# adajel/KNP-EMI-DG

Hardware: AMD Instinct MI355X
Metric: DoF-updates/sec per PDE timestep (higher is better)
Workload: dtype f64; 1 GPU; 3D idealized 4-axon mesh r=2 (995328 tets, 11943936 P1-DG DoFs: phi + K,Cl solved, Na eliminated), HH membranes + stimulus, full splitting step; parallelism=slab1

## Files before the change

### knp-emi-dg_amd/csrc/apply_ring.hip

```cpp
#include "cell_geom.hpp"
#include "ring_common.hpp"
#include "ring_facet.hpp"
#include <algorithm>
#include <cstdlib>
#include <map>

namespace {

using namespace ring;
constexpr int RH = 224;
constexpr int RHX = RH / 32;
constexpr int RENT = RB + RH;
constexpr int RSLOTS = 3;
constexpr int RLISTB = 1024;
constexpr int RNLIST = 4;
constexpr int RLOADERS = 4;
constexpr int META_F = 0, META_L = 1024, META_N = 3072, META_C = 4096, META_M = 5120, META_KNP = 6144, META_EMI = 5120;
constexpr int RCLS = 43;

__device__ __forceinline__ void dma_list(const MeshDev& m, int64_t b, unsigned dst, int lane) {
    const int off = lane * 4 < m.hb_stride ? lane * 4 : 0;
    glds16(m.hb_src + b * m.hb_stride + off, dst);
}
template <int NTHREADS> __device__ __forceinline__ void stage_class_records(const MeshDev& m, double* s_cls) {
    for (int i = threadIdx.x; i < m.ncls * 11; i += NTHREADS) s_cls[(i / 11) * RCLS + (i % 11)] = m.cls_table[(i / 11) * KNP_CLS_STRIDE + (i % 11)];
    for (int i = threadIdx.x; i < m.ncls * KNP_CLS_EXT; i += NTHREADS) s_cls[(i / KNP_CLS_EXT) * RCLS + 11 + (i % KNP_CLS_EXT)] = m.cls_ext[i];
}

template <int NS> struct KnpRing {
    static constexpr int XB = RENT * 32;
    static constexpr int G0 = NS * XB;
    static constexpr int GH0 = G0 + RB * 32;
    static constexpr int META0 = GH0 + 4096;
    static constexpr int SLOT = META0 + META_KNP;
    static constexpr int NDATA = NS * 8 + NS * RHX + 8 + 4 + 6;
    static_assert(NDATA <= 63, "vmcnt is a 6-bit counter");
};

struct CellMeta { uint32_t flags, nm; uint2 lw; unsigned cls, mymat; };
__device__ __forceinline__ CellMeta read_meta(const char* meta, unsigned t, bool knp) {
    CellMeta q;
    q.flags = ((const lds_u32*)(meta + META_F))[t];
    q.lw.x = ((const lds_u32*)(meta + META_L))[2 * t];
    q.lw.y = ((const lds_u32*)(meta + META_L))[2 * t + 1];
    q.cls = ((const lds_u16*)(meta + META_C))[t];
    q.nm = 0; q.mymat = 0;
    if (knp) {
        q.nm = ((const lds_u32*)(meta + META_N))[t];
        q.mymat = ((const lds_u8*)(meta + META_M))[t];
    }
    return q;
}

template <int NS, int NG>
__global__ __launch_bounds__(RB * NG + 64 * RLOADERS) void k_knp_apply_ring(MeshDev m, const double* __restrict__ x, const double* __restrict__ gphi,
                                                                 double* __restrict__ yout, KnpArgs ka, const uint8_t* __restrict__ mat,
                                                                 const uint8_t* __restrict__ nmat4, const double* __restrict__ dtab, int dbg) {
    typedef KnpRing<NS> R;
    constexpr int NV = 4, KS = NS / NG, NTHREADS = RB * NG + 64 * RLOADERS;
    static_assert(KS * NG == NS, "species split evenly over the consumer groups");
    extern __shared__ __attribute__((aligned(16))) char smem[];
    char* s_list = smem + RSLOTS * R::SLOT;
    double* s_cls = reinterpret_cast<double*>(s_list + RNLIST * RLISTB);
    double* s_D = s_cls + m.ncls * RCLS;
    const unsigned base = __builtin_amdgcn_readfirstlane((unsigned)(size_t)(lds_char*)smem);
    const unsigned list0 = base + RSLOTS * R::SLOT;
    const int wave = __builtin_amdgcn_readfirstlane((int)(threadIdx.x >> 6));
    const int lane = threadIdx.x & 63;
    const RingWalk w(m);
    if (w.blk(0) < 0) return;
    stage_class_records<NTHREADS>(m, s_cls);
    if (threadIdx.x < NS * KNP_MAX_MAT) s_D[threadIdx.x] = dtab[threadIdx.x];
    if (wave >= 4 * NG) {
        const int lw = wave - 4 * NG;
        constexpr int N0 = 8 + 3, N1 = (NS > 1 ? 8 : 0) + 3, N2 = 8 + 4, N3 = NS * RHX;
        auto list_dma = [&](int64_t n) {
            const int64_t b = w.blk(n);
            if (lw == 0 && b >= 0) dma_list(m, b, list0 + (unsigned)(n & (RNLIST - 1)) * RLISTB, lane);
        };
        auto data_dma = [&](int64_t n) {
            const int64_t b = w.blk(n);
            if (dbg & 4) return;
            const unsigned slot = base + (unsigned)(n % RSLOTS) * R::SLOT;
            const lds_int* L = (const lds_int*)(s_list + (n & (RNLIST - 1)) * RLISTB);
            const int64_t c0 = b * RB;
            if (lw == 0) {
                dma_own_rows(x, c0, m.nc, slot, lane);
                glds16(m.fflag + c0 + 4 * lane, slot + R::META0 + META_F);
                glds16(m.hb_loc + (c0 + 2 * lane) * 4, slot + R::META0 + META_L);
                glds16(m.hb_loc + (c0 + 128 + 2 * lane) * 4, slot + R::META0 + META_L + 1024);
            } else if (lw == 1) {
                if (NS > 1) dma_own_rows(x + m.nc * NV, c0, m.nc, slot + R::XB, lane);
                glds16(m.cls + c0 + 8 * lane, slot + R::META0 + META_C);
                glds16(nmat4 + (c0 + 4 * lane) * 4, slot + R::META0 + META_N);
                glds16(mat + c0 + 16 * lane, slot + R::META0 + META_M);
            } else if (lw == 2) {
                dma_own_rows(gphi, c0, m.nc, slot + R::G0, lane);
#pragma unroll
                for (int p = 0; p < 4; ++p) {
                    const int e = p * 64 + lane;
                    const int src = e < m.hb_stride ? L[e] : -1;
                    int64_t Kp = src >= 0 ? (int64_t)(src >> 2) : 0;
                    const int j = src >= 0 ? (src & 3) : 0;
                    if (dbg & 1) Kp = c0 + e < m.nc ? c0 + e : 0;
                    glds16(gphi + Kp * NV + (j >> 1) * 2, slot + R::GH0 + p * 1024);
                }
            } else {
#pragma unroll
                for (int p = 0; p < RHX; ++p) {
                    int64_t Kp = list_cell(L, p * 32 + (lane >> 1), m.hb_stride);
                    if (dbg & 1) Kp = c0 + p * 32 + (lane >> 1) < m.nc ? c0 + p * 32 + (lane >> 1) : 0;
#pragma unroll
                    for (int k = 0; k < NS; ++k) glds16(x + (int64_t)k * m.nc * NV + Kp * NV + swz_half(lane), slot + k * R::XB + RB * 32 + p * 1024);
                }
            }
        };
        load_two_ahead_counted<false, N0, N1, N2, N3>(w, lw, list_dma, data_dma);
        return;
    }
    const unsigned t = threadIdx.x & (RB - 1);
    const int k0 = (wave >> 2) * KS;
    double zpsi[KS];
#pragma unroll
    for (int k = 0; k < KS; ++k) zpsi[k] = ka.z[k0 + k] * ka.psi;
    ring_barrier();
    ring_barrier();
    for (int64_t n = 0;; ++n) {
        const int64_t b = w.blk(n);
        if (b < 0) break;
        const int64_t c = b * RB + t;
        if (c >= m.c_begin && c < m.c_end) {
            const char* slot = smem + (n % RSLOTS) * R::SLOT;
            const CellMeta cur = read_meta(slot + R::META0, t, true);
            const lds_double* X = (const lds_double*)slot + k0 * (RENT * NV);
            const lds_double* G = (const lds_double*)(slot + R::G0);
            const lds_double* rec = TO_LDS(s_cls) + cur.cls * RCLS;
            const lds_double* sD = TO_LDS(s_D) + k0 * KNP_MAX_MAT;
            CellGeom<3> K;
            class_gram<3>(rec, K);
            double xv[KS][NV], y[KS][NV], gp[NV], Dk[KS];
            lds_row(G, t, gp);
#pragma unroll
            for (int k = 0; k < KS; ++k) {
                lds_row(X + k * (RENT * NV), t, xv[k]);
                Dk[k] = sD[k * KNP_MAX_MAT + cur.mymat];
            }
            double gx[KS][NV], hvD[KS];
            knp_cell_term<KS>(K, xv, gp, Dk, zpsi, ka.inv_dt, gx, hvD, y);
            const ClassCoef ft{rec + 11};
            if (!(dbg & 2)) {
            knp_facet_ring<KS, 0, RENT * NV>(K, cur.flags, cur.lw.x & 0xffffu, ft, cur.nm & 0xffu, xv, gx, gp, Dk, hvD, zpsi, ka.tau, X, G, sD, y);
            knp_facet_ring<KS, 1, RENT * NV>(K, cur.flags, cur.lw.x >> 16, ft, (cur.nm >> 8) & 0xffu, xv, gx, gp, Dk, hvD, zpsi, ka.tau, X, G, sD, y);
            knp_facet_ring<KS, 2, RENT * NV>(K, cur.flags, cur.lw.y & 0xffffu, ft, (cur.nm >> 16) & 0xffu, xv, gx, gp, Dk, hvD, zpsi, ka.tau, X, G, sD, y);
            knp_facet_ring<KS, 3, RENT * NV>(K, cur.flags, cur.lw.y >> 16, ft, cur.nm >> 24, xv, gx, gp, Dk, hvD, zpsi, ka.tau, X, G, sD, y);
            }
#pragma unroll
            for (int k = 0; k < KS; ++k) store_nodal<3>(yout + (int64_t)(k0 + k) * m.nc * NV, c, y[k]);
        }
        ring_barrier();
    }
}

struct EmiRing {
    static constexpr int XB = RENT * 32;
    static constexpr int META0 = 2 * XB;
    static constexpr int SLOT = META0 + META_EMI;
    static constexpr int NDATA = 8 + 8 + 2 * RHX + 4;
};

constexpr int EMI_SLOTS = 4;
__global__ __launch_bounds__(2 * RB + 64 * RLOADERS) void k_emi_apply_ring(MeshDev m, const double* __restrict__ x, const double* __restrict__ kappa,
                                                                double* __restrict__ yout, double C_phi, double tau) {
    typedef EmiRing R;
    constexpr int NV = 4, NTHREADS = 2 * RB + 64 * RLOADERS;
    extern __shared__ __attribute__((aligned(16))) char smem[];
    char* s_list = smem + EMI_SLOTS * R::SLOT;
    double* s_cls = reinterpret_cast<double*>(s_list + RNLIST * RLISTB);
    const unsigned base = __builtin_amdgcn_readfirstlane((unsigned)(size_t)(lds_char*)smem);
    const unsigned list0 = base + EMI_SLOTS * R::SLOT;
    const int wave = __builtin_amdgcn_readfirstlane((int)(threadIdx.x >> 6));
    const int lane = threadIdx.x & 63;
    const RingWalk w(m);
    if (w.blk(0) < 0) return;
    stage_class_records<NTHREADS>(m, s_cls);
    if (wave >= 8) {
        const int lw = wave - 8;
        constexpr int N0 = 8, N1 = 8, N2 = RHX + 2, N3 = RHX + 2;
        auto list_dma = [&](int64_t n) {
            const int64_t b = w.blk(n);
            if (lw == 0 && b >= 0) dma_list(m, b, list0 + (unsigned)(n & (RNLIST - 1)) * RLISTB, lane);
        };
        auto data_dma = [&](int64_t n) {
            const int64_t c0 = w.blk(n) * RB;
            const unsigned slot = base + (unsigned)(n & (EMI_SLOTS - 1)) * R::SLOT;
            const lds_int* L = (const lds_int*)(s_list + (n & (RNLIST - 1)) * RLISTB);
            if (lw == 0) dma_own_rows(x, c0, m.nc, slot, lane);
            else if (lw == 1) dma_own_rows(kappa, c0, m.nc, slot + R::XB, lane);
            else {
                const double* v = lw == 2 ? x : kappa;
                const unsigned dst = slot + (lw == 2 ? 0 : R::XB) + RB * 32;
#pragma unroll
                for (int p = 0; p < RHX; ++p) glds16(v + list_cell(L, p * 32 + (lane >> 1), m.hb_stride) * NV + swz_half(lane), dst + p * 1024);
                if (lw == 2) {
                    glds16(m.fflag + c0 + 4 * lane, slot + R::META0 + META_F);
                    glds16(m.cls + c0 + 8 * lane, slot + R::META0 + META_C);
                } else {
                    glds16(m.hb_loc + (c0 + 2 * lane) * 4, slot + R::META0 + META_L);
                    glds16(m.hb_loc + (c0 + 128 + 2 * lane) * 4, slot + R::META0 + META_L + 1024);
                }
            }
        };
        load_two_ahead_counted<true, N0, N1, N2, N3>(w, lw, list_dma, data_dma);
        return;
    }
    const unsigned t = threadIdx.x & (RB - 1);
    const int g = wave >> 2;
    ring_barrier();
    ring_barrier();
    CellGeom<3> K;
    double xv[NV], kv[NV], yv[NV], gx[NV];
    const lds_double *X = nullptr, *KA = nullptr;
    ClassCoef ft{nullptr};
    CellMeta cur;
    cur.flags = 0; cur.lw = make_uint2(0u, 0u); cur.cls = 0; cur.nm = 0; cur.mymat = 0;
    int64_t ccur = -1;
    bool valid = false;
    for (int64_t n = 0;; ++n) {
        const int64_t b = w.blk(n);
        if ((n & 1) == g) {
            if (b >= 0) {
                ccur = b * RB + t;
                valid = ccur >= m.c_begin && ccur < m.c_end;
                if (valid) {
                    const char* slot = smem + (n & (EMI_SLOTS - 1)) * R::SLOT;
                    cur = read_meta(slot + R::META0, t, false);
                    X = (const lds_double*)slot;
                    KA = (const lds_double*)(slot + R::XB);
                    const lds_double* rec = TO_LDS(s_cls) + cur.cls * RCLS;
                    ft.ft = rec + 11;
                    class_gram<3>(rec, K);
                    lds_row(X, t, xv);
                    lds_row(KA, t, kv);
                    emi_cell_term(K, xv, kv, gx, yv);
                    emi_facet_ring<0>(K, cur.flags, cur.lw.x & 0xffffu, ft, xv, gx, kv, C_phi, tau, X, KA, yv);
                    emi_facet_ring<1>(K, cur.flags, cur.lw.x >> 16, ft, xv, gx, kv, C_phi, tau, X, KA, yv);
                }
            }
        } else if (n >= 1 && valid) {
            emi_facet_ring<2>(K, cur.flags, cur.lw.y & 0xffffu, ft, xv, gx, kv, C_phi, tau, X, KA, yv);
            emi_facet_ring<3>(K, cur.flags, cur.lw.y >> 16, ft, xv, gx, kv, C_phi, tau, X, KA, yv);
            store_nodal<3>(yout, ccur, yv);
        }
        ring_barrier();
        if (b < 0) break;
    }
}

}

static size_t ring_lds_bytes(const knp_ctx* c, int which) {
    const size_t tables = RNLIST * RLISTB + sizeof(double) * (size_t)c->m.ncls * RCLS;
    if (which == 0) return (size_t)EMI_SLOTS * EmiRing::SLOT + tables;
    const size_t slot = c->p.n_sys == 1 ? KnpRing<1>::SLOT : KnpRing<2>::SLOT;
    return (size_t)RSLOTS * slot + tables + sizeof(double) * (size_t)c->p.n_sys * KNP_MAX_MAT;
}

bool ring_usable(const knp_ctx* c, int which) {
    if (c->degree != 1 || c->m.dim != 3 || !c->m.cls || c->m.ncls > CLS_MAX_LDS || !c->m.hb_src || c->m.hb_stride <= 0 || c->m.hb_stride > RH) return false;
    if (env_int("KNP_APPLY_RING", 1) == 0 || ring_lds_bytes(c, which) > RING_MAX_LDS) return false;
    if (which == 0) return env_int("KNP_EMI_RING", 1) != 0;
    return c->nmat > 0 && c->p.n_sys <= 2 && env_int("KNP_APPLY_MAT", 1) != 0 && env_int("KNP_APPLY_HALO", 1) != 0;
}

int ring_emi_apply(knp_ctx* c, const MeshDev& m, const double* x, const double* kappa, double* y, int reserve_cus) {
    const size_t lds = ring_lds_bytes(c, 0);
    if (!grant_lds(c, k_emi_apply_ring, lds)) { c->err = "hipFuncSetAttribute(k_emi_apply_ring) failed"; return -2; }
    hipLaunchKernelGGL(k_emi_apply_ring, ring_grid(c, m, reserve_cus), dim3(2 * RB + 64 * RLOADERS), lds, c->stream, m, x, kappa, y, c->p.C_phi, c->p.tau_emi);
    HIPCHK(c, hipGetLastError());
    return 0;
}

int ring_knp_apply(knp_ctx* c, const MeshDev& m, const double* x, const double* gphi, double* y, const KnpArgs& ka, int reserve_cus) {
    const int ns = c->p.n_sys;
    const size_t lds = ring_lds_bytes(c, 1);
    const dim3 g = ring_grid(c, m, reserve_cus);
    const bool split = ns == 2 && env_int("KNP_RING_SPLIT", 0) != 0;
#define RING_KNP_LAUNCH(NS_, NG_)                                                                                                     \
    do {                                                                                                                              \
        if (!grant_lds(c, k_knp_apply_ring<NS_, NG_>, lds)) { c->err = "hipFuncSetAttribute(k_knp_apply_ring) failed"; return -2; }  \
        hipLaunchKernelGGL((k_knp_apply_ring<NS_, NG_>), g, dim3(RB * NG_ + 64 * RLOADERS), lds, c->stream, m, x, gphi, y, ka, (const uint8_t*)c->mat,  \
                           (const uint8_t*)c->nmat4, (const double*)c->dtab, env_int("KNP_RING_DEBUG", 0));                     \
    } while (0)
    if (ns == 1) RING_KNP_LAUNCH(1, 1);
    else if (split) RING_KNP_LAUNCH(2, 2);
    else RING_KNP_LAUNCH(2, 1);
#undef RING_KNP_LAUNCH
    HIPCHK(c, hipGetLastError());
    return 0;
}
```

### knp-emi-dg_amd/csrc/ring_facet.hpp

```cpp
#pragma once
#include "ring_common.hpp"

namespace ring {


struct ClassCoef {
    const lds_double* ft;
    template <int I> __device__ __forceinline__ double area(const CellGeom<3>&) const { return ft[8 * I + 6]; }
    template <int I> __device__ __forceinline__ void coef(const CellGeom<3>&, double& gr, double* cf, double& pen_geo, double& nLI_DV) const {
        gr = ft[8 * I];
        pen_geo = ft[8 * I + 4];
        nLI_DV = ft[8 * I + 5];
#pragma unroll
        for (int mm = 0; mm < 3; ++mm) cf[mm] = ft[8 * I + 1 + mm];
    }
};

__device__ __forceinline__ void lds_vertex(const lds_double* co, unsigned v, double* X) {
    typedef double __attribute__((ext_vector_type(2))) vdouble2;
    typedef __attribute__((address_space(3))) vdouble2 lds_vdouble2;
    const vdouble2 a = *(const lds_vdouble2*)(co + 4 * v);
    X[0] = a.x; X[1] = a.y; X[2] = co[4 * v + 2];
}
struct CoordCoef {
    const lds_double* co;
    unsigned vapex;
    double hinv;
    template <int I> __device__ __forceinline__ double area(const CellGeom<3>& K) const { return fast_sqrt(K.G[I][I]) * (3.0 * K.vol); }
    template <int I> __device__ __forceinline__ void coef(const CellGeom<3>& K, double& gr, double* cf, double& pen_geo, double& nLI_DV) const {
        double Xo[3], L[4];
        lds_vertex(co, vapex, Xo);
        apex_bary<3>(K, Xo, L);
        gr = K.G[I][I] * fast_rcp(L[I]);
#pragma unroll
        for (int mm = 0; mm < 3; ++mm) cf[mm] = fma(-L[mm + (mm >= I)], gr, K.G[mm + (mm >= I)][I]);
        const double DV = 3.0 * K.vol;
        pen_geo = hinv * area<I>(K);
        nLI_DV = -L[I] * DV;
    }
};

__device__ __forceinline__ void emi_cell_term(const CellGeom<3>& K, const double* xv, const double* kv, double* gx, double* y) {
    constexpr int NV = 4;
    double kbar = 0.0;
#pragma unroll
    for (int a = 0; a < NV; ++a) kbar += kv[a];
    kbar *= K.vol / (double)NV;
#pragma unroll
    for (int a = 0; a < NV; ++a) {
        double sa = 0.0;
#pragma unroll
        for (int bb = 0; bb < NV; ++bb) sa = fma(xv[bb], K.G[bb][a], sa);
        gx[a] = sa;
        y[a] = kbar * sa;
    }
}

template <int I, typename Coef>
__device__ __forceinline__ void emi_facet_ring(const CellGeom<3>& K, uint32_t flags, unsigned loc, const Coef& src, const double* xv, const double* gx,
                                               const double* kv, double C_phi, double tau, const lds_double* X, const lds_double* KA, double* y) {
    constexpr int D = 3, NV = 4;
    const uint32_t fb = (flags >> (8 * I)) & 0xffu;
    const uint32_t kind = (fb >> 2) & 3u;
    if (kind >= FK_EXTERIOR) return;
    const unsigned j = fb & 3u;
    double xr[NV], kr[NV], xf[D], knf[D];
    lds_row(X, loc, xr);
    lds_row(KA, loc, kr);
    const double xap = pick_apex<D>(xr, (int)j);
#pragma unroll
    for (int mm = 0; mm < D; ++mm) {
        xf[mm] = pick_facet<D>(xr, mm, (int)j);
        knf[mm] = pick_facet<D>(kr, mm, (int)j);
    }
    double du[D], sdu = 0.0;
#pragma unroll
    for (int mm = 0; mm < D; ++mm) {
        du[mm] = xv[mm + (mm >= I)] - xf[mm];
        sdu += du[mm];
    }
    if (kind == FK_MEMBRANE) {
        const double w = C_phi * src.template area<I>(K) * FacetConst<D>::mass;
#pragma unroll
        for (int mm = 0; mm < D; ++mm) y[mm + (mm >= I)] = fma(w, sdu + du[mm], y[mm + (mm >= I)]);
        return;
    }
    double gr, cf[D], pen_geo, nLI_DV;
    src.template coef<I>(K, gr, cf, pen_geo, nLI_DV);
    const double s_own = gx[I];
    double s_nb = xap * gr;
#pragma unroll
    for (int mm = 0; mm < D; ++mm) s_nb = fma(xf[mm], cf[mm], s_nb);
    double kf[D], sk = 0.0, skn = 0.0, q = 0.0;
#pragma unroll
    for (int mm = 0; mm < D; ++mm) {
        kf[mm] = kv[mm + (mm >= I)];
        sk += kf[mm];
        skn += knf[mm];
        q = fma(kf[mm], sdu + du[mm], q);
    }
    const double hm = 0.5 * (double)D * K.vol * FacetConst<D>::mass;
    q *= hm;
#pragma unroll
    for (int a = 0; a < NV; ++a) y[a] = fma(K.G[a][I], q, y[a]);
    const double pw = tau * pen_geo * FacetConst<D>::trip;
    double kb[D], skb = 0.0, skd = 0.0;
#pragma unroll
    for (int mm = 0; mm < D; ++mm) {
        kb[mm] = 0.5 * (kf[mm] + knf[mm]);
        skb += kb[mm];
        skd = fma(kb[mm], du[mm], skd);
    }
    const double bs = fma(skb, sdu, skd);
#pragma unroll
    for (int mm = 0; mm < D; ++mm) {
        const double t1 = hm * fma(s_own, sk + kf[mm], s_nb * (skn + knf[mm]));
        const double t3 = pw * (bs + fma(kb[mm], sdu, du[mm] * fma(2.0, kb[mm], skb)));
        y[mm + (mm >= I)] += t1 + t3;
    }
}

template <int NS>
__device__ __forceinline__ void knp_cell_term(const CellGeom<3>& K, const double (*xv)[4], const double* gp, const double* Dk, const double* zpsi,
                                              double inv_dt, double (*gx)[4], double* hvD, double (*y)[4]) {
    constexpr int NV = 4;
    const double mw = inv_dt * K.vol / 20.0;
#pragma unroll
    for (int k = 0; k < NS; ++k) hvD[k] = 0.5 * K.vol * Dk[k];
#pragma unroll
    for (int k = 0; k < NS; ++k) {
        double sx = 0.0;
#pragma unroll
        for (int a = 0; a < NV; ++a) sx += xv[k][a];
        const double drift = zpsi[k] * Dk[k] * K.vol * sx / (double)NV;
        const double dv = Dk[k] * K.vol;
#pragma unroll
        for (int a = 0; a < NV; ++a) {
            double sacc = 0.0;
#pragma unroll
            for (int bb = 0; bb < NV; ++bb) sacc = fma(xv[k][bb], K.G[bb][a], sacc);
            gx[k][a] = sacc;
            y[k][a] = fma(mw, sx + xv[k][a], fma(dv, sacc, drift * gp[a]));
        }
    }
}

template <int NS, int I, int XS, typename Coef>
__device__ __forceinline__ void knp_facet_ring(const CellGeom<3>& K, uint32_t flags, unsigned loc, const Coef& src, unsigned dsel, const double (*xv)[4],
                                               const double (*gx)[4], const double* gp, const double* Dk, const double* hvD, const double* zpsi,
                                               double tau, const lds_double* X, const lds_double* G, const lds_double* sD, double (*y)[4]) {
    constexpr int D = 3, NV = 4;
    const uint32_t fb = (flags >> (8 * I)) & 0xffu;
    if (((fb >> 2) & 3u) != FK_SIPG) return;
    const unsigned j = fb & 3u;
    double gr, cf[D], pen_geo, nLI_DV;
    src.template coef<I>(K, gr, cf, pen_geo, nLI_DV);
    double gp_nb;
    {
        typedef double __attribute__((ext_vector_type(2))) vdouble2;
        typedef __attribute__((address_space(3))) vdouble2 lds_vdouble2;
        const unsigned idx = loc < (unsigned)RB ? loc * NV + 2u * (((j >> 1) ^ (loc >> 3)) & 1u) : (unsigned)(RB * NV) + (loc - RB) * 2u;
        const vdouble2 g2 = *(const lds_vdouble2*)(G + idx);
        gp_nb = (j & 1u) ? g2.y : g2.x;
    }
    const double DV = (double)D * K.vol;
    const double up_own = fmax(-gp[I], 0.0) * DV;
    const double up_nb = fmax(-gp_nb, 0.0) * nLI_DV;
    const double penA = tau * pen_geo;
    const double hv = 0.5 * K.vol;
#pragma unroll
    for (int k = 0; k < NS; ++k) {
        double xr[NV], xf[D];
        lds_row(X + (unsigned)k * XS, loc, xr);
        const double xap = pick_apex<D>(xr, (int)j);
#pragma unroll
        for (int mm = 0; mm < D; ++mm) xf[mm] = pick_facet<D>(xr, mm, (int)j);
        const double Dn = sD[(unsigned)k * KNP_MAX_MAT + dsel];
        const double s_own = gx[k][I];
        double s_nb = xap * gr;
#pragma unroll
        for (int mm = 0; mm < D; ++mm) s_nb = fma(xf[mm], cf[mm], s_nb);
        const double zp = zpsi[k];
        const double c_own = Dk[k] * fma(-zp, up_own, penA);
        const double c_nb = Dn * fma(-zp, up_nb, penA);
        double sdu = 0.0, w[D], sw = 0.0;
#pragma unroll
        for (int mm = 0; mm < D; ++mm) {
            const double xo = xv[k][mm + (mm >= I)];
            sdu += xo - xf[mm];
            w[mm] = fma(c_own, xo, -c_nb * xf[mm]);
            sw += w[mm];
        }
        const double t1m = fma(FacetConst<D>::mass, sw, hv * fma(Dk[k], s_own, Dn * s_nb));
        const double t2 = hvD[k] * sdu;
#pragma unroll
        for (int a = 0; a < NV; ++a) y[k][a] = fma(K.G[a][I], t2, y[k][a]);
#pragma unroll
        for (int mm = 0; mm < D; ++mm) y[k][mm + (mm >= I)] += fma(FacetConst<D>::mass, w[mm], t1m);
    }
}

}
```

Measured before the change: 2.255 billion DoF/s.

## Software-pipeline LDS neighbor loads ahead of facet compute in ring apply kernels

Splits the KNP and EMI facet routines into a load phase (neighbor rows, diffusion coefficients, class coefficients read from LDS into registers) and a compute phase, then issues each facet's loads one facet ahead of the previous facet's arithmetic. Loads are now issued unconditionally, using the cell's own row when the facet is inactive. The loader waves also read all list entries up front before issuing the global-to-LDS copies, and hoist the swizzle offset. The aim is to hide LDS latency behind the FMA work, at the cost of more registers and possibly lower occupancy.

New measurement: 2.251 billion DoF/s. About the same (-0.2%).

```diff
diff --git a/knp-emi-dg_amd/csrc/apply_ring.hip b/knp-emi-dg_amd/csrc/apply_ring.hip
--- a/knp-emi-dg_amd/csrc/apply_ring.hip
+++ b/knp-emi-dg_amd/csrc/apply_ring.hip
@@ -21,6 +21,17 @@
 __device__ __forceinline__ void dma_list(const MeshDev& m, int64_t b, unsigned dst, int lane) {
     const int off = lane * 4 < m.hb_stride ? lane * 4 : 0;
     glds16(m.hb_src + b * m.hb_stride + off, dst);
+}
+template <int N, int STEP> __device__ __forceinline__ void list_entries(const lds_int* L, int e0, int hs, int* src) {
+    static_assert((N - 1) * STEP + 64 <= RLISTB / 4, "list reads stay inside the list buffer");
+#pragma unroll
+    for (int p = 0; p < N; ++p) src[p] = L[e0 + p * STEP];
+#pragma unroll
+    for (int p = 0; p < N; ++p) src[p] = e0 + p * STEP < hs ? src[p] : -1;
+}
+template <int N, int STEP> __device__ __forceinline__ void own_entries(int64_t c0, int e0, int64_t nc, int* src) {
+#pragma unroll
+    for (int p = 0; p < N; ++p) src[p] = c0 + e0 + p * STEP < nc ? (int)(c0 + e0 + p * STEP) << 2 : 0;
 }
 template <int NTHREADS> __device__ __forceinline__ void stage_class_records(const MeshDev& m, double* s_cls) {
     for (int i = threadIdx.x; i < m.ncls * 11; i += NTHREADS) s_cls[(i / 11) * RCLS + (i % 11)] = m.cls_table[(i / 11) * KNP_CLS_STRIDE + (i % 11)];
@@ -50,6 +61,21 @@
         q.mymat = ((const lds_u8*)(meta + META_M))[t];
     }
     return q;
+}
+
+__device__ __forceinline__ unsigned meta_loc(const CellMeta& q, int I) { return ((I < 2 ? q.lw.x : q.lw.y) >> (16 * (I & 1))) & 0xffffu; }
+template <int KS, int I>
+__device__ __forceinline__ void knp_facet_load(const CellMeta& q, unsigned t, const lds_double* ft, const lds_double* X, const lds_double* G,
+                                               const lds_double* sD, KnpFacetRows<KS>& r, ClassCoef& fc) {
+    const bool on = facet_kind(q.flags, I) == FK_SIPG;
+    fc.load<I>(ft);
+    knp_facet_rows<KS, RENT * 4>(on ? meta_loc(q, I) : t, (q.flags >> (8 * I)) & 3u, on ? (q.nm >> (8 * I)) & 0xffu : q.mymat, X, G, sD, r);
+}
+template <int I>
+__device__ __forceinline__ void emi_facet_load(const CellMeta& q, unsigned t, const lds_double* ft, const lds_double* X, const lds_double* KA,
+                                               EmiFacetRows& r, ClassCoef& fc) {
+    fc.load<I>(ft);
+    emi_facet_rows(facet_kind(q.flags, I) < FK_EXTERIOR ? meta_loc(q, I) : t, X, KA, r);
 }
 
 template <int NS, int NG>
@@ -78,6 +104,7 @@
             const int64_t b = w.blk(n);
             if (lw == 0 && b >= 0) dma_list(m, b, list0 + (unsigned)(n & (RNLIST - 1)) * RLISTB, lane);
         };
+        const double* xrow = x + swz_half(lane);
         auto data_dma = [&](int64_t n) {
             const int64_t b = w.blk(n);
             if (dbg & 4) return;
@@ -96,22 +123,24 @@
                 glds16(mat + c0 + 16 * lane, slot + R::META0 + META_M);
             } else if (lw == 2) {
                 dma_own_rows(gphi, c0, m.nc, slot + R::G0, lane);
+                int src[4];
+                list_entries<4, 64>(L, lane, m.hb_stride, src);
+                if (dbg & 1) own_entries<4, 64>(c0, lane, m.nc, src);
 #pragma unroll
                 for (int p = 0; p < 4; ++p) {
-                    const int e = p * 64 + lane;
-                    const int src = e < m.hb_stride ? L[e] : -1;
-                    int64_t Kp = src >= 0 ? (int64_t)(src >> 2) : 0;
-                    const int j = src >= 0 ? (src & 3) : 0;
-                    if (dbg & 1) Kp = c0 + e < m.nc ? c0 + e : 0;
+                    const int64_t Kp = src[p] >= 0 ? (int64_t)(src[p] >> 2) : 0;
+                    const int j = src[p] >= 0 ? (src[p] & 3) : 0;
                     glds16(gphi + Kp * NV + (j >> 1) * 2, slot + R::GH0 + p * 1024);
                 }
             } else {
+                int src[RHX];
+                list_entries<RHX, 32>(L, lane >> 1, m.hb_stride, src);
+                if (dbg & 1) own_entries<RHX, 32>(c0, lane >> 1, m.nc, src);
 #pragma unroll
                 for (int p = 0; p < RHX; ++p) {
-                    int64_t Kp = list_cell(L, p * 32 + (lane >> 1), m.hb_stride);
-                    if (dbg & 1) Kp = c0 + p * 32 + (lane >> 1) < m.nc ? c0 + p * 32 + (lane >> 1) : 0;
-#pragma unroll
-                    for (int k = 0; k < NS; ++k) glds16(x + (int64_t)k * m.nc * NV + Kp * NV + swz_half(lane), slot + k * R::XB + RB * 32 + p * 1024);
+                    const int64_t Kp = src[p] >= 0 ? (int64_t)(src[p] >> 2) : 0;
+#pragma unroll
+                    for (int k = 0; k < NS; ++k) glds16(xrow + (int64_t)k * m.nc * NV + Kp * NV, slot + k * R::XB + RB * 32 + p * 1024);
                 }
             }
         };
@@ -145,14 +174,20 @@
                 lds_row(X + k * (RENT * NV), t, xv[k]);
                 Dk[k] = sD[k * KNP_MAX_MAT + cur.mymat];
             }
+            KnpFacetRows<KS> nb[4];
+            ClassCoef fc[4];
+            const bool facets = !(dbg & 2);
+            if (facets) knp_facet_load<KS, 0>(cur, t, rec + 11, X, G, sD, nb[0], fc[0]);
             double gx[KS][NV], hvD[KS];
             knp_cell_term<KS>(K, xv, gp, Dk, zpsi, ka.inv_dt, gx, hvD, y);
-            const ClassCoef ft{rec + 11};
-            if (!(dbg & 2)) {
-            knp_facet_ring<KS, 0, RENT * NV>(K, cur.flags, cur.lw.x & 0xffffu, ft, cur.nm & 0xffu, xv, gx, gp, Dk, hvD, zpsi, ka.tau, X, G, sD, y);
-            knp_facet_ring<KS, 1, RENT * NV>(K, cur.flags, cur.lw.x >> 16, ft, (cur.nm >> 8) & 0xffu, xv, gx, gp, Dk, hvD, zpsi, ka.tau, X, G, sD, y);
-            knp_facet_ring<KS, 2, RENT * NV>(K, cur.flags, cur.lw.y & 0xffffu, ft, (cur.nm >> 16) & 0xffu, xv, gx, gp, Dk, hvD, zpsi, ka.tau, X, G, sD, y);
-            knp_facet_ring<KS, 3, RENT * NV>(K, cur.flags, cur.lw.y >> 16, ft, cur.nm >> 24, xv, gx, gp, Dk, hvD, zpsi, ka.tau, X, G, sD, y);
+            if (facets) {
+                knp_facet_load<KS, 1>(cur, t, rec + 11, X, G, sD, nb[1], fc[1]);
+                if (facet_kind(cur.flags, 0) == FK_SIPG) knp_facet_terms<KS, 0>(K, cur.flags, fc[0], nb[0], xv, gx, gp, Dk, hvD, zpsi, ka.tau, y);
+                knp_facet_load<KS, 2>(cur, t, rec + 11, X, G, sD, nb[2], fc[2]);
+                if (facet_kind(cur.flags, 1) == FK_SIPG) knp_facet_terms<KS, 1>(K, cur.flags, fc[1], nb[1], xv, gx, gp, Dk, hvD, zpsi, ka.tau, y);
+                knp_facet_load<KS, 3>(cur, t, rec + 11, X, G, sD, nb[3], fc[3]);
+                if (facet_kind(cur.flags, 2) == FK_SIPG) knp_facet_terms<KS, 2>(K, cur.flags, fc[2], nb[2], xv, gx, gp, Dk, hvD, zpsi, ka.tau, y);
+                if (facet_kind(cur.flags, 3) == FK_SIPG) knp_facet_terms<KS, 3>(K, cur.flags, fc[3], nb[3], xv, gx, gp, Dk, hvD, zpsi, ka.tau, y);
             }
 #pragma unroll
             for (int k = 0; k < KS; ++k) store_nodal<3>(yout + (int64_t)(k0 + k) * m.nc * NV, c, y[k]);
@@ -197,10 +232,12 @@
             if (lw == 0) dma_own_rows(x, c0, m.nc, slot, lane);
             else if (lw == 1) dma_own_rows(kappa, c0, m.nc, slot + R::XB, lane);
             else {
-                const double* v = lw == 2 ? x : kappa;
+                const double* v = (lw == 2 ? x : kappa) + swz_half(lane);
                 const unsigned dst = slot + (lw == 2 ? 0 : R::XB) + RB * 32;
-#pragma unroll
-                for (int p = 0; p < RHX; ++p) glds16(v + list_cell(L, p * 32 + (lane >> 1), m.hb_stride) * NV + swz_half(lane), dst + p * 1024);
+                int src[RHX];
+                list_entries<RHX, 32>(L, lane >> 1, m.hb_stride, src);
+#pragma unroll
+                for (int p = 0; p < RHX; ++p) glds16(v + (src[p] >= 0 ? (int64_t)(src[p] >> 2) : 0) * NV, dst + p * 1024);
                 if (lw == 2) {
                     glds16(m.fflag + c0 + 4 * lane, slot + R::META0 + META_F);
                     glds16(m.cls + c0 + 8 * lane, slot + R::META0 + META_C);
@@ -219,8 +256,9 @@
     ring_barrier();
     CellGeom<3> K;
     double xv[NV], kv[NV], yv[NV], gx[NV];
-    const lds_double *X = nullptr, *KA = nullptr;
-    ClassCoef ft{nullptr};
+    EmiFacetRows nb[4];
+    ClassCoef fc[4];
+    const lds_double *X3 = nullptr, *rec3 = nullptr;
     CellMeta cur;
     cur.flags = 0; cur.lw = make_uint2(0u, 0u); cur.cls = 0; cur.nm = 0; cur.mymat = 0;
     int64_t ccur = -1;
@@ -234,21 +272,25 @@
                 if (valid) {
                     const char* slot = smem + (n & (EMI_SLOTS - 1)) * R::SLOT;
                     cur = read_meta(slot + R::META0, t, false);
-                    X = (const lds_double*)slot;
-                    KA = (const lds_double*)(slot + R::XB);
+                    const lds_double* X = (const lds_double*)slot;
+                    const lds_double* KA = (const lds_double*)(slot + R::XB);
                     const lds_double* rec = TO_LDS(s_cls) + cur.cls * RCLS;
-                    ft.ft = rec + 11;
+                    X3 = X; rec3 = rec + 11;
                     class_gram<3>(rec, K);
                     lds_row(X, t, xv);
                     lds_row(KA, t, kv);
+                    emi_facet_load<0>(cur, t, rec + 11, X, KA, nb[0], fc[0]);
                     emi_cell_term(K, xv, kv, gx, yv);
-                    emi_facet_ring<0>(K, cur.flags, cur.lw.x & 0xffffu, ft, xv, gx, kv, C_phi, tau, X, KA, yv);
-                    emi_facet_ring<1>(K, cur.flags, cur.lw.x >> 16, ft, xv, gx, kv, C_phi, tau, X, KA, yv);
+                    emi_facet_load<1>(cur, t, rec + 11, X, KA, nb[1], fc[1]);
+                    if (facet_kind(cur.flags, 0) < FK_EXTERIOR) emi_facet_terms<0>(K, cur.flags, fc[0], nb[0], xv, gx, kv, C_phi, tau, yv);
+                    emi_facet_load<2>(cur, t, rec + 11, X, KA, nb[2], fc[2]);
+                    if (facet_kind(cur.flags, 1) < FK_EXTERIOR) emi_facet_terms<1>(K, cur.flags, fc[1], nb[1], xv, gx, kv, C_phi, tau, yv);
                 }
             }
         } else if (n >= 1 && valid) {
-            emi_facet_ring<2>(K, cur.flags, cur.lw.y & 0xffffu, ft, xv, gx, kv, C_phi, tau, X, KA, yv);
-            emi_facet_ring<3>(K, cur.flags, cur.lw.y >> 16, ft, xv, gx, kv, C_phi, tau, X, KA, yv);
+            emi_facet_load<3>(cur, t, rec3, X3, X3 + R::XB / 8, nb[3], fc[3]);
+            if (facet_kind(cur.flags, 2) < FK_EXTERIOR) emi_facet_terms<2>(K, cur.flags, fc[2], nb[2], xv, gx, kv, C_phi, tau, yv);
+            if (facet_kind(cur.flags, 3) < FK_EXTERIOR) emi_facet_terms<3>(K, cur.flags, fc[3], nb[3], xv, gx, kv, C_phi, tau, yv);
             store_nodal<3>(yout, ccur, yv);
         }
         ring_barrier();
diff --git a/knp-emi-dg_amd/csrc/ring_facet.hpp b/knp-emi-dg_amd/csrc/ring_facet.hpp
--- a/knp-emi-dg_amd/csrc/ring_facet.hpp
+++ b/knp-emi-dg_amd/csrc/ring_facet.hpp
@@ -5,16 +5,21 @@
 
 
 struct ClassCoef {
-    const lds_double* ft;
-    template <int I> __device__ __forceinline__ double area(const CellGeom<3>&) const { return ft[8 * I + 6]; }
+    double v[7];
+    template <int I> __device__ __forceinline__ void load(const lds_double* ft) {
+#pragma unroll
+        for (int i = 0; i < 7; ++i) v[i] = ft[8 * I + i];
+    }
+    template <int I> __device__ __forceinline__ double area(const CellGeom<3>&) const { return v[6]; }
     template <int I> __device__ __forceinline__ void coef(const CellGeom<3>&, double& gr, double* cf, double& pen_geo, double& nLI_DV) const {
-        gr = ft[8 * I];
-        pen_geo = ft[8 * I + 4];
-        nLI_DV = ft[8 * I + 5];
-#pragma unroll
-        for (int mm = 0; mm < 3; ++mm) cf[mm] = ft[8 * I + 1 + mm];
+        gr = v[0];
+        pen_geo = v[4];
+        nLI_DV = v[5];
+#pragma unroll
+        for (int mm = 0; mm < 3; ++mm) cf[mm] = v[1 + mm];
     }
 };
+__device__ __forceinline__ uint32_t facet_kind(uint32_t flags, int I) { return (flags >> (8 * I + 2)) & 3u; }
 
 __device__ __forceinline__ void lds_vertex(const lds_double* co, unsigned v, double* X) {
     typedef double __attribute__((ext_vector_type(2))) vdouble2;
@@ -56,17 +61,20 @@
     }
 }
 
+struct EmiFacetRows { double xr[4], kr[4]; };
+__device__ __forceinline__ void emi_facet_rows(unsigned loc, const lds_double* X, const lds_double* KA, EmiFacetRows& r) {
+    lds_row(X, loc, r.xr);
+    lds_row(KA, loc, r.kr);
+}
 template <int I, typename Coef>
-__device__ __forceinline__ void emi_facet_ring(const CellGeom<3>& K, uint32_t flags, unsigned loc, const Coef& src, const double* xv, const double* gx,
-                                               const double* kv, double C_phi, double tau, const lds_double* X, const lds_double* KA, double* y) {
+__device__ __forceinline__ void emi_facet_terms(const CellGeom<3>& K, uint32_t flags, const Coef& src, const EmiFacetRows& r, const double* xv,
+                                                const double* gx, const double* kv, double C_phi, double tau, double* y) {
     constexpr int D = 3, NV = 4;
     const uint32_t fb = (flags >> (8 * I)) & 0xffu;
     const uint32_t kind = (fb >> 2) & 3u;
-    if (kind >= FK_EXTERIOR) return;
     const unsigned j = fb & 3u;
-    double xr[NV], kr[NV], xf[D], knf[D];
-    lds_row(X, loc, xr);
-    lds_row(KA, loc, kr);
+    const double *xr = r.xr, *kr = r.kr;
+    double xf[D], knf[D];
     const double xap = pick_apex<D>(xr, (int)j);
 #pragma unroll
     for (int mm = 0; mm < D; ++mm) {
@@ -118,6 +126,14 @@
         const double t3 = pw * (bs + fma(kb[mm], sdu, du[mm] * fma(2.0, kb[mm], skb)));
         y[mm + (mm >= I)] += t1 + t3;
     }
+}
+template <int I, typename Coef>
+__device__ __forceinline__ void emi_facet_ring(const CellGeom<3>& K, uint32_t flags, unsigned loc, const Coef& src, const double* xv, const double* gx,
+                                               const double* kv, double C_phi, double tau, const lds_double* X, const lds_double* KA, double* y) {
+    if (facet_kind(flags, I) >= FK_EXTERIOR) return;
+    EmiFacetRows r;
+    emi_facet_rows(loc, X, KA, r);
+    emi_facet_terms<I>(K, flags, src, r, xv, gx, kv, C_phi, tau, y);
 }
 
 template <int NS>
@@ -145,24 +161,33 @@
     }
 }
 
-template <int NS, int I, int XS, typename Coef>
-__device__ __forceinline__ void knp_facet_ring(const CellGeom<3>& K, uint32_t flags, unsigned loc, const Coef& src, unsigned dsel, const double (*xv)[4],
-                                               const double (*gx)[4], const double* gp, const double* Dk, const double* hvD, const double* zpsi,
-                                               double tau, const lds_double* X, const lds_double* G, const lds_double* sD, double (*y)[4]) {
-    constexpr int D = 3, NV = 4;
-    const uint32_t fb = (flags >> (8 * I)) & 0xffu;
-    if (((fb >> 2) & 3u) != FK_SIPG) return;
-    const unsigned j = fb & 3u;
-    double gr, cf[D], pen_geo, nLI_DV;
-    src.template coef<I>(K, gr, cf, pen_geo, nLI_DV);
-    double gp_nb;
+template <int NS> struct KnpFacetRows { double xr[NS][4], g2[2], Dn[NS]; };
+template <int NS, int XS>
+__device__ __forceinline__ void knp_facet_rows(unsigned loc, unsigned j, unsigned dsel, const lds_double* X, const lds_double* G, const lds_double* sD,
+                                               KnpFacetRows<NS>& r) {
+    constexpr int NV = 4;
     {
         typedef double __attribute__((ext_vector_type(2))) vdouble2;
         typedef __attribute__((address_space(3))) vdouble2 lds_vdouble2;
         const unsigned idx = loc < (unsigned)RB ? loc * NV + 2u * (((j >> 1) ^ (loc >> 3)) & 1u) : (unsigned)(RB * NV) + (loc - RB) * 2u;
         const vdouble2 g2 = *(const lds_vdouble2*)(G + idx);
-        gp_nb = (j & 1u) ? g2.y : g2.x;
-    }
+        r.g2[0] = g2.x; r.g2[1] = g2.y;
+    }
+#pragma unroll
+    for (int k = 0; k < NS; ++k) {
+        lds_row(X + (unsigned)k * XS, loc, r.xr[k]);
+        r.Dn[k] = sD[(unsigned)k * KNP_MAX_MAT + dsel];
+    }
+}
+template <int NS, int I, typename Coef>
+__device__ __forceinline__ void knp_facet_terms(const CellGeom<3>& K, uint32_t flags, const Coef& src, const KnpFacetRows<NS>& r, const double (*xv)[4],
+                                                const double (*gx)[4], const double* gp, const double* Dk, const double* hvD, const double* zpsi,
+                                                double tau, double (*y)[4]) {
+    constexpr int D = 3, NV = 4;
+    const unsigned j = (flags >> (8 * I)) & 3u;
+    double gr, cf[D], pen_geo, nLI_DV;
+    src.template coef<I>(K, gr, cf, pen_geo, nLI_DV);
+    const double gp_nb = (j & 1u) ? r.g2[1] : r.g2[0];
     const double DV = (double)D * K.vol;
     const double up_own = fmax(-gp[I], 0.0) * DV;
     const double up_nb = fmax(-gp_nb, 0.0) * nLI_DV;
@@ -170,12 +195,12 @@
     const double hv = 0.5 * K.vol;
 #pragma unroll
     for (int k = 0; k < NS; ++k) {
-        double xr[NV], xf[D];
-        lds_row(X + (unsigned)k * XS, loc, xr);
+        const double* xr = r.xr[k];
+        double xf[D];
         const double xap = pick_apex<D>(xr, (int)j);
 #pragma unroll
         for (int mm = 0; mm < D; ++mm) xf[mm] = pick_facet<D>(xr, mm, (int)j);
-        const double Dn = sD[(unsigned)k * KNP_MAX_MAT + dsel];
+        const double Dn = r.Dn[k];
         const double s_own = gx[k][I];
         double s_nb = xap * gr;
 #pragma unroll
@@ -199,5 +224,14 @@
         for (int mm = 0; mm < D; ++mm) y[k][mm + (mm >= I)] += fma(FacetConst<D>::mass, w[mm], t1m);
     }
 }
-
-}
+template <int NS, int I, int XS, typename Coef>
+__device__ __forceinline__ void knp_facet_ring(const CellGeom<3>& K, uint32_t flags, unsigned loc, const Coef& src, unsigned dsel, const double (*xv)[4],
+                                               const double (*gx)[4], const double* gp, const double* Dk, const double* hvD, const double* zpsi,
+                                               double tau, const lds_double* X, const lds_double* G, const lds_double* sD, double (*y)[4]) {
+    if (facet_kind(flags, I) != FK_SIPG) return;
+    KnpFacetRows<NS> r;
+    knp_facet_rows<NS, XS>(loc, (flags >> (8 * I)) & 3u, dsel, X, G, sD, r);
+    knp_facet_terms<NS, I>(K, flags, src, r, xv, gx, gp, Dk, hvD, zpsi, tau, y);
+}
+
+}
```
